# epam/Zstandard

Measured on AMD Instinct MI355X. Metric: GiB/s compress @ level 3, 64 KiB chunks, higher is better.
Workload: dtype u8; 1 GPU; 4096 independent 65536 B chunks per GPU per step, level 3, BASELINE config[1] shape (Silesia unavailable offline -> Zipf-token log stream, SURVEY 8d); chunks_per_gpu=4096, chunk_bytes=65536, level=3, parallelism=chunks sharded over 1 GPU(s), no collective in the data path

## Files before the change

### zstandard_amd/csrc/lz_kernels.hip

```cpp
#include "zsmi_device.h"
#include "zsmi_scratch.h"
#include <type_traits>

#ifndef ZS_CAND_G
#define ZS_CAND_G 8
#endif
#ifndef ZS_CAND_G_BIG
#define ZS_CAND_G_BIG 16
#endif
#define ZS_CAND_GOF(TLOG) ((TLOG) > ZS_TABLE_LOG_SMALL ? ZS_CAND_G_BIG : ZS_CAND_G)
#ifndef ZS_CAND_DEPTH
#define ZS_CAND_DEPTH 2
#endif
#define ZS_CAND_WAVES(NT) (3 * (NT))
#define ZS_CAND_ROW 65u
#define ZS_CAND_LDS(TLOG, NT) ((size_t)(NT) * (4u << (TLOG)) + 3u * (NT) * ZS_CAND_GOF(TLOG) * ZS_CAND_ROW * 4u + (NT) * 256u + 3u * 16u * 8u + 32u)
#define ZS_SLOT_EMPTY 0xFFFFFFFFu
__device__ __forceinline__ uint32_t zs_hash_short(uint32_t lo, uint32_t hi) { return __umul24(lo, 0x9E3779u) + __umul24(__builtin_amdgcn_alignbit(hi, lo, 16), 0x85EBCBu); }
__device__ __forceinline__ uint32_t zs_hash_long(uint32_t lo, uint32_t hi)
{ return __umul24(lo, 0x9E3779u) + __umul24(__builtin_amdgcn_alignbit(hi, lo, 24), 0x85EBCBu) + __umul24(hi >> 16, 0xC2B2AFu); }

template <int TLOG, int NT, bool PFX = false>
__global__ void __launch_bounds__(64 * ZS_CAND_WAVES(NT))
k_lz_candidates(const uint8_t *__restrict__ src, const ZsUnitDesc *__restrict__ units, uint32_t block0,
                uint16_t *__restrict__ distAll, uint8_t *__restrict__ distHiAll, uint32_t *__restrict__ candCount,
                const ZsCDictEntry *__restrict__ dictTab = nullptr, const uint32_t *__restrict__ unitDict = nullptr,
                const uint32_t *__restrict__ liveUnits = nullptr)
{
    static_assert(!PFX || TLOG == ZS_TABLE_LOG_BIG, "a prefixed unit spans up to 128 KiB of positions");
    if (liveUnits && blockIdx.x >= *liveUnits) return;
    const uint32_t *dictImg = nullptr; uint32_t pfx = 0;
    if constexpr (PFX) {
        const ZsCDictEntry &de = dictTab[unitDict ? unitDict[blockIdx.x] : 0u];
        dictImg = de.img; pfx = (uint32_t)__builtin_amdgcn_readfirstlane((int)de.pfx);
    }
    extern __shared__ __attribute__((aligned(16))) uint32_t candLds[];
    constexpr bool BIG = TLOG > ZS_TABLE_LOG_SMALL;
    constexpr uint32_t G = ZS_CAND_GOF(TLOG), GP = G * 64u, H = G / NT;
    constexpr uint32_t M = ZS_CAND_DEPTH;
    constexpr uint32_t LPS = 64u / G;
    constexpr uint32_t WD = G / 4u + 2u;
    static_assert(G == 8 || G == 16, "a hasher lane takes G consecutive positions of a group: 8 or 16");
    const uint32_t wave = (uint32_t)__builtin_amdgcn_readfirstlane((int)(threadIdx.x >> 6)), lane = threadIdx.x & 63u;
    const uint32_t tab = (wave < NT) ? wave : ((wave < 2 * NT) ? wave - NT : wave - 2 * NT);
    uint32_t *T = candLds + ((size_t)tab << TLOG);
    uint32_t *opnd = candLds + ((size_t)NT << TLOG);
    constexpr uint32_t ROW = ZS_CAND_ROW, GR = G * ROW;
    constexpr uint32_t RING = 3u * NT * GR;
    uint64_t *runMarks = reinterpret_cast<uint64_t *>(opnd + RING + NT * 64u);
    uint32_t *runFlag = opnd + RING + NT * 64u + 3u * 16u * 2u;
    const ZsUnitDesc ud = units[blockIdx.x];
    const uint8_t *s = src + ud.srcOff;
    const uint32_t n = ud.size;
    const size_t slot = (size_t)(ud.firstBlock - block0);
    uint16_t *dist = zs_block_dist(distAll, slot);
    uint8_t *distHi = zs_block_dist_hi(distHiAll, slot);
    const uint32_t hashable = (n >= 8) ? n - 7 : 0;
    const uint32_t nGroups = (hashable + GP - 1) / GP;
    if (threadIdx.x < 2) zs_block_cand(candCount, slot, threadIdx.x) = 0;
    if (nGroups == 0) return;
    if (n >= 16 && (n & 15u) == 0) {
        uint4 f;
        __builtin_memcpy(&f, s, 16);
        const uint32_t splat = (f.x & 0xFFu) * 0x01010101u;
        if (((f.x ^ splat) | (f.y ^ splat) | (f.z ^ splat) | (f.w ^ splat)) == 0) {
            if (threadIdx.x == 0) candLds[0] = 0;
            __syncthreads();
            uint32_t mixed = 0;
            for (uint32_t i = threadIdx.x * 16u; i < n && !mixed; i += ZS_CAND_WAVES(NT) * 64u * 16u) {
                uint4 v;
                __builtin_memcpy(&v, s + i, 16);
                mixed = (v.x ^ splat) | (v.y ^ splat) | (v.z ^ splat) | (v.w ^ splat);
            }
            if (mixed) candLds[0] = 1u;
            __syncthreads();
            const bool uniform = candLds[0] == 0;
            __syncthreads();
            if (uniform) return;
        }
    }
    const uint32_t dummyBase = ((uint32_t)(NT - tab) << TLOG) + RING + tab * 64u;
    auto mergeRead = [&](uint32_t g, uint32_t (&mS)[H], uint32_t (&mL)[H]) {
        const uint32_t *xb = opnd + (size_t)(g % 3u) * NT * GR + (NT > 1 ? tab * H : 0u) * ROW + lane;
        #pragma unroll
        for (uint32_t uu = 0; uu < H; uu++) { mS[uu] = xb[uu * ROW]; mL[uu] = (NT > 1) ? xb[GR + uu * ROW] : 0u; }
    };
    uint32_t found = 0;
    const uint32_t matchlessBelow = n >> ZS_MATCHLESS_SHIFT;
    auto mergeStore = [&](uint32_t g, const uint32_t (&mS)[H], const uint32_t (&mL)[H]) {
        const uint32_t sbase = g * GP + ((NT > 1) ? tab * H * 64u : 0u);
        uint64_t hiMine = 0;
        #pragma unroll
        for (uint32_t uu = 0; uu < H; uu++) {
            const uint32_t dm = (NT > 1) ? (mL[uu] ? mL[uu] : mS[uu]) : mS[uu];
            if (BIG) { const uint64_t hi = __ballot((dm >> 16) != 0); if (lane == uu) hiMine = hi; }
            if (found < matchlessBelow) {
                if ((g + 1u) * GP <= hashable) found += (uint32_t)__popcll(__ballot(dm != 0));
                else found += (uint32_t)__popcll(__ballot(dm != 0 && sbase + uu * 64 + lane < hashable));
            }
            dist[sbase + uu * 64 + lane] = (uint16_t)dm;
        }
        if (BIG && lane < H) *reinterpret_cast<uint64_t *>(distHi + ((sbase + lane * 64) >> 3)) = hiMine;
    };
    if (wave >= 2 * NT) {
        __syncthreads(); __syncthreads();
        for (uint32_t i = 2; i <= nGroups + 1; i++) {
            uint32_t mS[H], mL[H];
            mergeRead(i - 2, mS, mL);
            if (__builtin_amdgcn_readfirstlane((int)runFlag[((i - 2) % 3u) * 2u + tab])) {
                if (lane == 0) runFlag[((i - 2) % 3u) * 2u + tab] = 0;
                #pragma unroll
                for (uint32_t uu = 0; uu < H; uu++) {
                    const uint64_t marks = runMarks[((i - 2) % 3u) * 16u + ((NT > 1) ? tab * H : 0u) + uu];
                    if ((marks >> lane) & 1ull) { if (NT > 1) mL[uu] = 1u; else mS[uu] = 1u; }
                }
            }
            mergeStore(i - 2, mS, mL);
            __syncthreads();
        }
        if (lane == 0) zs_block_cand(candCount, slot, tab) = found;
        return;
    }

    if (wave < NT) {
        if constexpr (PFX) {
            uint4 *t4 = reinterpret_cast<uint4 *>(T);
            const uint4 *img4 = reinterpret_cast<const uint4 *>(dictImg + ((size_t)tab << TLOG));
            #pragma unroll 8
            for (uint32_t i = lane; i < (1u << TLOG) / 4; i += 64) t4[i] = img4[i];
        } else {
            uint4 *t4 = reinterpret_cast<uint4 *>(T);
            const uint4 e = make_uint4(ZS_SLOT_EMPTY, ZS_SLOT_EMPTY, ZS_SLOT_EMPTY, ZS_SLOT_EMPTY);
            #pragma unroll 8
            for (uint32_t i = lane; i < (1u << TLOG) / 4; i += 64) t4[i] = e;
        }
        uint32_t ringSlot = 0;
        __syncthreads();
        for (uint32_t i = 1; i <= nGroups; i++) {
            uint32_t *ob = opnd + ((size_t)ringSlot * NT + tab) * GR + lane;
            const uint32_t base = (i - 1) * GP + lane + (PFX ? pfx : 0u);
            uint32_t op[G], entry[G], old[G];
            #pragma unroll
            for (uint32_t u = 0; u < G; u++) op[u] = ob[u * ROW];
            #pragma unroll
            for (uint32_t u = 0; u < G; u++) {
                uint32_t pu = base + u * 64u;
                asm volatile("" : "+v"(pu));
                entry[u] = (op[u] & 0xFFFE0000u) | pu;
                old[u] = atomicExch(&T[op[u] & 0xFFFFu], entry[u]);
            }
            #pragma unroll
            for (uint32_t u = 0; u < G; u++) {
                const uint32_t x = old[u] ^ entry[u], dd = entry[u] - old[u];
                ob[u * ROW] = (max(x, dd) < (1u << 17)) ? dd : 0u;
            }
            ringSlot = (ringSlot == 2u) ? 0u : ringSlot + 1u;
            __syncthreads();
        }
        __syncthreads();
        return;
    }

    auto run = [&](auto roleTag) {
        constexpr bool LONG = decltype(roleTag)::value;
        const uint32_t stepOfLane = lane / LPS, l0 = (lane % LPS) * G;
        const uint32_t wbase = stepOfLane * ROW + l0;
        const uint32_t last8 = n - 8;
        auto loadGroup = [&](uint32_t g, uint32_t (&w)[WD]) {
            const uint32_t o = g * GP + lane * G;
            #pragma unroll
            for (uint32_t k = 0; k < WD / 2; k++) {
                const uint32_t ok = o + 8u * k, oc = min(ok, last8);
                const uint64_t v = zs_load64(s + oc) >> (8u * min(ok - oc, 7u));
                w[2 * k] = (uint32_t)v; w[2 * k + 1] = (uint32_t)(v >> 32);
            }
        };
        uint32_t bufA[M][WD], bufB[M][WD];
        auto loadM = [&](uint32_t g0, uint32_t (&buf)[M][WD]) {
            #pragma unroll
            for (uint32_t k = 0; k < M; k++) loadGroup(min(g0 + k, nGroups), buf[k]);
        };
        auto iter = [&](auto wholeTag, uint32_t i, const uint32_t (&w)[WD]) {
            constexpr bool WHOLE = decltype(wholeTag)::value;
            const uint32_t ringSlot = i % 3u;
            if (i < nGroups) {
                uint32_t *ob = opnd + ((size_t)ringSlot * NT + tab) * GR + wbase;
                const uint32_t pbase = i * GP + lane * G;
                #pragma unroll
                for (uint32_t u = 0; u < G; u++) {
                    const uint32_t k = u >> 2, sh = u & 3u;
                    const uint32_t lo = sh ? __builtin_amdgcn_alignbyte(w[k + 1], w[k], sh) : w[k];
                    const uint32_t hi = sh ? __builtin_amdgcn_alignbyte(w[min(k + 2, WD - 1)], w[k + 1], sh) : w[k + 1];
                    uint32_t h = LONG ? zs_hash_long(lo, hi) : zs_hash_short(lo, hi);
                    asm volatile("" : "+v"(h));
                    const uint32_t r = __builtin_amdgcn_alignbit(h, h, 32 - TLOG);
                    ob[u] = (WHOLE || pbase + u < hashable) ? (r & (0xFFFE0000u | ((1u << TLOG) - 1u))) : ((r & 0xFFFE0000u) | (dummyBase + l0 + u));
                }
                bool flat = false;
                uint64_t flatLanes = 0;
                if (WHOLE && __ballot(w[0] == w[1])) {
                    uint32_t diff = w[0] ^ __builtin_amdgcn_alignbyte(w[0], w[0], 1);
                    #pragma unroll
                    for (uint32_t k = 1; k < WD; k++) diff |= w[k] ^ w[k - 1];
                    flat = diff == 0;
                    flatLanes = __ballot(flat);
                }
                if (flatLanes) {
                    const uint32_t key = flat ? ((w[0] & 0xFFu) | 0x100u) : 0u;
                    const uint32_t keyBelow = (uint32_t)__builtin_amdgcn_update_dpp(0, (int)key, 0x138, 0xF, 0xF, true);
                    const uint32_t keyAbove = (uint32_t)__builtin_amdgcn_update_dpp(0, (int)key, 0x130, 0xF, 0xF, true);
                    const bool markFirst = flat && keyBelow == key && (lane % LPS) != 0u;
                    const bool innerLast = flat && keyAbove == key && (lane % LPS) != LPS - 1u;
                    if (flat) {
                        uint32_t h = LONG ? zs_hash_long(w[0], w[1]) : zs_hash_short(w[0], w[1]);
                        asm volatile("" : "+v"(h));
                        const uint32_t away = (__builtin_amdgcn_alignbit(h, h, 32 - TLOG) & 0xFFFE0000u) | (dummyBase + l0);
                        if (markFirst) ob[0] = away;
                        #pragma unroll
                        for (uint32_t u = 1; u + 1 < G; u++) ob[u] = away + u;
                        if (innerLast) ob[G - 1] = away + (G - 1);
                    }
                    if (!LONG) {
                        if (lane < NT) runFlag[ringSlot * 2u + lane] = 1u;
                        const uint32_t bits = flat ? (((1u << G) - 2u) | (markFirst ? 1u : 0u)) : 0u;
                        if (G == 8) reinterpret_cast<uint8_t *>(runMarks + ringSlot * 16u)[lane] = (uint8_t)bits;
                        else reinterpret_cast<uint16_t *>(runMarks + ringSlot * 16u)[lane] = (uint16_t)bits;
                    }
                }
            }
            __syncthreads();
        };
        auto step = [&](uint32_t i, const uint32_t (&w)[WD]) {
            if (i > nGroups + 1) return;
            if ((i + 1) * GP + 8u <= n) iter(std::true_type{}, i, w); else iter(std::false_type{}, i, w);
        };
        if (!LONG && lane < 6u) runFlag[lane] = 0;
        loadM(0, bufA);
        for (uint32_t g0 = 0; g0 <= nGroups + 1; g0 += 2 * M) {
            loadM(g0 + M, bufB);
            #pragma unroll
            for (uint32_t k = 0; k < M; k++) step(g0 + k, bufA[k]);
            loadM(g0 + 2 * M, bufA);
            #pragma unroll
            for (uint32_t k = 0; k < M; k++) step(g0 + M + k, bufB[k]);
        }
    };
    if (tab == 0) run(std::false_type{}); else run(std::true_type{});
}

__global__ void __launch_bounds__(1024)
k_lz_dict_tables(const ZsCDictEntry entry, ZsCDictEntry *__restrict__ entryOut)
{
    constexpr int TLOG = ZS_TABLE_LOG_BIG;
    __shared__ uint32_t T[1u << TLOG];
    const uint32_t tab = blockIdx.x, tid = threadIdx.x;
    const uint8_t *__restrict__ pre = entry.pre; const uint32_t pfx = entry.pfx; uint32_t *__restrict__ img = const_cast<uint32_t *>(entry.img);
    if (tab == 0 && tid == 0) *entryOut = entry;
    for (uint32_t i = tid; i < (1u << TLOG); i += 1024) T[i] = 0;
    __syncthreads();
    const uint32_t hashable = pfx >= 8 ? pfx - 7 : 0;
    for (uint32_t p = tid; p < hashable; p += 1024) {
        const uint64_t v = zs_load64(pre + p);
        const uint32_t lo = (uint32_t)v, hi = (uint32_t)(v >> 32);
        const uint32_t h = tab ? zs_hash_long(lo, hi) : zs_hash_short(lo, hi);
        const uint32_t r = __builtin_amdgcn_alignbit(h, h, 32 - TLOG);
        atomicMax(&T[r & ((1u << TLOG) - 1u)], ((p + 1u) << 15) | (r >> 17));
    }
    __syncthreads();
    uint32_t *out = img + ((size_t)tab << TLOG);
    for (uint32_t i = tid; i < (1u << TLOG); i += 1024) {
        const uint32_t k = T[i];
        out[i] = k ? (((k & 0x7FFFu) << 17) | ((k >> 15) - 1u)) : ZS_SLOT_EMPTY;
    }
}

#ifndef ZS_WALK_MINW
#define ZS_WALK_MINW 1
#endif
#define ZS_WALK_WGRP(WLOG) ((WLOG) >= 9 ? 4 : 2)
#ifndef ZS_WALK_LPW_256
#define ZS_WALK_LPW_256 2
#endif
#ifndef ZS_WALK_LPW_512
#define ZS_WALK_LPW_512 4
#endif
#define ZS_WALK_LPW(WLOG) ((WLOG) >= 9 ? ZS_WALK_LPW_512 : ZS_WALK_LPW_256)
#define ZS_WALK_THREADS(BIG, WLOG) ((((BIG) ? ZS_UNIT_MAX : ZS_BLOCK_MAX) >> (WLOG)) * ZS_WALK_LPW(WLOG))
static_assert(ZS_WALK_THREADS(false, 8) / ZS_WALK_LPW(8) == (ZS_BLOCK_MAX >> 8) && ZS_WALK_THREADS(false, 9) / ZS_WALK_LPW(9) == (ZS_BLOCK_MAX >> 9) &&
              ZS_WALK_THREADS(true, 8) / ZS_WALK_LPW(8) == (ZS_UNIT_MAX >> 8) && ZS_WALK_THREADS(true, 9) / ZS_WALK_LPW(9) == (ZS_UNIT_MAX >> 9),
              "a walker per walk range of a unit of full capacity");
#define ZS_WALK_KERNEL(LOOK, REPW, BIG, WLOG) k_lz_walk<ZS_WALK_LPW(WLOG), ZS_WALK_WGRP(WLOG), LOOK, REPW, BIG, ZS_WALK_THREADS(BIG, WLOG)>
#ifndef ZS_WALK_SKEW
#define ZS_WALK_SKEW  24u
#endif
#define ZS_WALK_FRONT 48u
#define ZS_WALK_TAIL  144u
#define ZS_WALK_SRCBYTES(CAPB) ((((CAPB) + ZS_WALK_TAIL + ZS_WALK_SKEW * (((CAPB) + ZS_WALK_TAIL) / 256u + 1u)) + 15u) & ~15u)
#define ZS_WALK_LDS(CAPB) ((CAPB) / 8 + 16 + ZS_WALK_FRONT + ZS_WALK_SRCBYTES(CAPB) + 16 + 1024)

typedef const __attribute__((address_space(3))) uint32_t *ZsLdsU32;
template <int K>
__device__ __forceinline__ void lds_span(uint32_t byteOff, uint32_t (&out)[K])
{
    ZsLdsU32 d = (ZsLdsU32)(uintptr_t)(byteOff & ~3u);
    uint32_t w[K + 1];
    #pragma unroll
    for (int k = 0; k <= K; k++) w[k] = d[k];
    const uint32_t sh = byteOff & 3u;
    #pragma unroll
    for (int k = 0; k < K; k++) out[k] = __builtin_amdgcn_alignbyte(w[k + 1], w[k], sh);
}
template <int I, int K>
__device__ __forceinline__ uint32_t span_at(const uint32_t (&v)[K])
{
    if constexpr ((I & 3) == 0) return v[I >> 2];
    else return __builtin_amdgcn_alignbyte(v[(I >> 2) + 1], v[I >> 2], I & 3);
}
__device__ __forceinline__ uint32_t zs_agree16(const uint32_t (&a)[4], const uint32_t (&b)[4])
{
    const uint64_t x0 = (uint64_t)(a[0] ^ b[0]) | ((uint64_t)(a[1] ^ b[1]) << 32), x1 = (uint64_t)(a[2] ^ b[2]) | ((uint64_t)(a[3] ^ b[3]) << 32);
    const uint32_t n0 = x0 ? ((uint32_t)__builtin_ctzll(x0) >> 3) : 8u;
    const uint32_t n1 = x1 ? ((uint32_t)__builtin_ctzll(x1) >> 3) : 8u;
    return (n0 < 8u) ? n0 : 8u + n1;
}
template <int LPW> __device__ __forceinline__ uint32_t walker_or(uint32_t v)
{
    if constexpr (LPW >= 2) v |= (uint32_t)__builtin_amdgcn_update_dpp(0, (int)v, 0xB1, 0xF, 0xF, false);
    if constexpr (LPW == 4) v |= (uint32_t)__builtin_amdgcn_update_dpp(0, (int)v, 0x4E, 0xF, 0xF, false);
    return v;
}
template <int LPW> __device__ __forceinline__ int walker_max(int v)
{
    if constexpr (LPW >= 2) v = max(v, __builtin_amdgcn_update_dpp(0, v, 0xB1, 0xF, 0xF, false));
    if constexpr (LPW == 4) v = max(v, __builtin_amdgcn_update_dpp(0, v, 0x4E, 0xF, 0xF, false));
    return v;
}
template <int LPW> __device__ __forceinline__ uint32_t walker_min(uint32_t v)
{
    if constexpr (LPW >= 2) v = min(v, (uint32_t)__builtin_amdgcn_update_dpp(0, (int)v, 0xB1, 0xF, 0xF, false));
    if constexpr (LPW == 4) v = min(v, (uint32_t)__builtin_amdgcn_update_dpp(0, (int)v, 0x4E, 0xF, 0xF, false));
    return v;
}
template <int NT, int DIR>
__device__ __forceinline__ uint32_t block_scan_max(uint32_t v, uint32_t *wv, uint32_t tid, uint32_t *total)
{
    const uint32_t lane = tid & 63u, wave = tid >> 6;
    #pragma unroll
    for (int d = 1; d < 64; d <<= 1) {
        const uint32_t o = (uint32_t)(DIR > 0 ? __shfl_up((int)v, d) : __shfl_down((int)v, d));
        if (DIR > 0 ? (int)lane >= d : (int)lane + d < 64) v = max(v, o);
    }
    __syncthreads();
    if (lane == (DIR > 0 ? 63u : 0u)) wv[wave] = v;
    __syncthreads();
    uint32_t pre = 0, all = 0;
    #pragma unroll
    for (uint32_t k = 0; k < NT / 64; k++) { const uint32_t x = wv[k]; all = max(all, x); if (DIR > 0 ? k < wave : k > wave) pre = max(pre, x); }
    *total = all;
    return max(v, pre);
}
__device__ __forceinline__ uint32_t zs_nonzero8(const uint4 d)
{
    typedef uint16_t u16x2 __attribute__((ext_vector_type(2)));
    const u16x2 one = { 1, 1 };
    (void)one;
    auto nz = [&](uint32_t w) { uint32_t r; asm("v_pk_min_u16 %0, %1, %2" : "=v"(r) : "v"(w), "v"(0x00010001u)); return r; };
    const uint32_t v = nz(d.x) | (nz(d.y) << 2) | (nz(d.z) << 4) | (nz(d.w) << 6);
    return (v | (v >> 15)) & 0xFFu;
}

#ifdef ZS_WALK_PROFILE
#define WPROF_STAMP(k) { __builtin_amdgcn_sched_barrier(0); unsigned long long t_; asm volatile("s_waitcnt vmcnt(0) lgkmcnt(0)\n\ts_memtime %0\n\ts_waitcnt lgkmcnt(0)" : "=s"(t_) :: "memory"); __builtin_amdgcn_sched_barrier(0); wprof[k] += t_ - wlast; wlast = t_; }
#else
#define WPROF_STAMP(k)
#endif
#define ZS_WALK_KERNEL_PFX(LOOK, REPW, WLOG) k_lz_walk<ZS_WALK_LPW(WLOG), ZS_WALK_WGRP(WLOG), LOOK, REPW, true, ZS_WALK_THREADS(false, WLOG), true>
template <int LPW, int WGRP, int LOOK, int REPWIN, bool BIG, int NT, bool PFX = false>
__global__ void __launch_bounds__(NT, BIG ? 1 : ZS_WALK_MINW)
k_lz_walk(const uint8_t *__restrict__ src, const ZsUnitDesc *__restrict__ units, uint32_t block0,
          const uint16_t *__restrict__ distAll, const uint8_t *__restrict__ distHiAll,
          uint2 *__restrict__ recAll, uint32_t junkSlot, uint4 *__restrict__ resAll, int rangeLogArg, const uint32_t *__restrict__ candCount,
          const ZsCDictEntry *__restrict__ dictTab = nullptr, const uint32_t *__restrict__ unitDict = nullptr,
          const uint32_t *__restrict__ liveUnits = nullptr)
{
    static_assert(!PFX || BIG, "a prefixed unit is staged in the 128 KiB layout");
    if (liveUnits && blockIdx.x >= *liveUnits) return;
    const uint8_t *pre = nullptr; uint32_t pfx = 0;
    if constexpr (PFX) {
        const ZsCDictEntry &de = dictTab[unitDict ? unitDict[blockIdx.x] : 0u];
        pre = de.pre; pfx = (uint32_t)__builtin_amdgcn_readfirstlane((int)de.pfx);
    }
    constexpr uint32_t CAP = BIG ? ZS_UNIT_MAX : ZS_BLOCK_MAX;
    constexpr uint32_t CPL = LOOK / LPW, RPL = REPWIN / LPW, GPL = WGRP / LPW;
    static_assert((LPW == 1 || LPW == 2 || LPW == 4) && WGRP % LPW == 0 && LOOK % LPW == 0 && REPWIN % LPW == 0 && CPL >= 1 && RPL >= 1 && LOOK <= 8 && REPWIN <= 8, "a walker's lanes share the groups and candidates evenly");
    static_assert(NT >= 64 && NT % 64 == 0 && NT * GPL * 16 <= CAP / 8, "the exchange buffer holds 16 bytes a lane and group");
    extern __shared__ __attribute__((aligned(16))) uint8_t walkLds[];
    constexpr uint32_t SRC = CAP / 8 + 16 + ZS_WALK_FRONT;
    auto lposv = [](uint32_t v) { return SRC + v + (uint32_t)__mul24((int)v >> 8, (int)ZS_WALK_SKEW); };
    const uint32_t vb = PFX ? pfx : 0u;
    auto lpos = [&](uint32_t p) { return lposv(p + vb); };
    auto stage16 = [&](uint32_t i, const uint4 v) {
        uint8_t *d = walkLds + lposv(i);
        *reinterpret_cast<uint2 *>(d) = make_uint2(v.x, v.y); *reinterpret_cast<uint2 *>(d + 8) = make_uint2(v.z, v.w);
        const uint32_t o = i & 255u;
        if (o == 0) { *reinterpret_cast<uint2 *>(d - ZS_WALK_SKEW) = make_uint2(v.x, v.y); *reinterpret_cast<uint2 *>(d - ZS_WALK_SKEW + 8) = make_uint2(v.z, v.w); }
        else if (o == 16) *reinterpret_cast<uint2 *>(d - ZS_WALK_SKEW) = make_uint2(v.x, v.y);
    };
    const uint32_t tid = threadIdx.x, lane = tid & 63u;
    const uint32_t rangeLog = (uint32_t)rangeLogArg, R = 1u << rangeLog;
    const ZsUnitDesc ud = units[blockIdx.x];
    const uint32_t slot = ud.firstBlock - block0;
    const uint8_t *s = src + ud.srcOff;
    const uint32_t n = ud.size;
    const uint16_t *dist = zs_block_dist(distAll, slot);
    const uint8_t *distHi = zs_block_dist_hi(distHiAll, slot);
    uint4 *xbuf = reinterpret_cast<uint4 *>(walkLds);
    const uint32_t xw = (tid & ~63u) * GPL;
    const uint32_t safeAddr = (xw + lane) * 16u;
    uint32_t *mixedWord = reinterpret_cast<uint32_t *>(walkLds + SRC + ZS_WALK_SRCBYTES(CAP)) + 1;
    uint4 *res = zs_block_range_results(resAll, slot);
    uint8_t *xhi = reinterpret_cast<uint8_t *>(mixedWord + 3);
    uint2 *recs = zs_block_walk_records(recAll, slot);
    const uint32_t sub = lane & (LPW - 1u);
#ifdef ZS_WALK_PROFILE
    unsigned long long wprof[10] = { 0, 0, 0, 0, 0, 0, 0, 0, 0, 0 }, wlast;
    asm volatile("s_memtime %0\n\ts_waitcnt lgkmcnt(0)" : "=s"(wlast) :: "memory");
#endif

    if (zs_block_cand(candCount, slot, 0) + zs_block_cand(candCount, slot, 1) < (n >> ZS_MATCHLESS_SHIFT)) {
        const uint32_t nRanges = (n + R - 1) >> rangeLog, perBlockLog = 16u - rangeLog;
        for (uint32_t r = tid; r < nRanges; r += NT) res[zs_unit_range_result(r, perBlockLog)] = make_uint4(0, 0, 0, 0);
        return;
    }
    uint32_t mixed = 0;
    if (tid < (ZS_WALK_FRONT - ZS_WALK_SKEW) / 4) reinterpret_cast<uint32_t *>(walkLds + SRC - ZS_WALK_FRONT)[tid] = 0;
    if (tid == 0) *mixedWord = 0;
    __syncthreads();
    if constexpr (PFX) {
        const uint32_t end = pfx + n, splat = (n ? (uint32_t)s[0] : 0u) * 0x01010101u;
        for (uint32_t i = tid * 16; i < end + ZS_WALK_TAIL && i + 16 <= CAP + ZS_WALK_TAIL; i += NT * 16) {
            uint4 w = make_uint4(0, 0, 0, 0);
            if (i + 16 <= pfx) __builtin_memcpy(&w, pre + i, 16);
            else if (i >= pfx && i + 16 <= end) {
                __builtin_memcpy(&w, s + (i - pfx), 16);
                mixed |= (w.x ^ splat) | (w.y ^ splat) | (w.z ^ splat) | (w.w ^ splat);
            } else if (i < end) {
                uint8_t b[16];
                for (uint32_t k = 0; k < 16; k++) {
                    const uint32_t v = i + k;
                    b[k] = v < pfx ? pre[v] : (v < end ? s[v - pfx] : (uint8_t)0);
                    if (v >= pfx && v < end && b[k] != (uint8_t)splat) mixed = 1;
                }
                __builtin_memcpy(&w, b, 16);
            }
            stage16(i, w);
        }
        if ((n & 15u) != 0 || n < 16) mixed = 1;
    } else {
        constexpr uint32_t PER = (CAP / 16 + NT - 1) / NT;
        const uint32_t nFull = n & ~15u;
        uint4 v[PER];
        const uint32_t splat = (n ? (uint32_t)s[0] : 0u) * 0x01010101u;
        #pragma unroll
        for (uint32_t k = 0; k < PER; k++) {
            const uint32_t i = (tid + k * NT) * 16;
            const uint32_t ii = (i + 16 <= nFull) ? i : 0u;
            v[k] = make_uint4(0, 0, 0, 0);
            if (nFull >= 16) __builtin_memcpy(&v[k], s + ii, 16);
        }
        #pragma unroll
        for (uint32_t k = 0; k < PER; k++) {
            const uint32_t i = (tid + k * NT) * 16;
            if (i + 16 <= nFull) stage16(i, v[k]);
            mixed |= (v[k].x ^ splat) | (v[k].y ^ splat) | (v[k].z ^ splat) | (v[k].w ^ splat);
        }
        if (n != nFull || n < 16) mixed = 1;
        for (uint32_t i = nFull + tid * 16; i < n + ZS_WALK_TAIL; i += NT * 16) {
            uint4 w = make_uint4(0, 0, 0, 0);
            if (i < n) {
                uint64_t lo = 0, hi = 0;
                for (uint32_t k = 0; k < 16 && i + k < n; k++) { const uint64_t c = s[i + k]; if (k < 8) lo |= c << (8 * k); else hi |= c << (8 * (k - 8)); }
                w = make_uint4((uint32_t)lo, (uint32_t)(lo >> 32), (uint32_t)hi, (uint32_t)(hi >> 32));
            }
            if (i + 16 <= CAP + ZS_WALK_TAIL) stage16(i, w);
        }
    }
#if defined(ZS_WALK_STOP) && ZS_WALK_STOP == 1
    if (n) return;
#endif
    const uint32_t hashable = (n >= 8) ? n - 7 : 0;
    if (mixed) *mixedWord = 1u;
    __syncthreads();
    if (*mixedWord == 0) {
        const uint32_t nRanges = (n + R - 1) >> rangeLog, perBlockLog = 16u - rangeLog;
        for (uint32_t r = tid; r < nRanges; r += NT) res[zs_unit_range_result(r, perBlockLog)] = make_uint4(0, 0, 0, 0);
        return;
    }
    WPROF_STAMP(0)

    {
        const uint32_t nRanges = (n + R - 1) >> rangeLog;
        bool active = false;
        uint32_t ip = 0, anchor = 0, scanEnd = 0, limit = 0, rep0 = 0, rep1 = 0, nseq = 0, lastOff = 0, blockBase = 0;
        uint2 heldRec = make_uint2(0, 0);
        const uint32_t perBlockLog = 16u - rangeLog;
        typedef __attribute__((address_space(3))) uint4 *ZsLdsU4;
        const uint32_t xwaveLds = (uint32_t)__builtin_amdgcn_readfirstlane((int)(uint32_t)(uintptr_t)(ZsLdsU4)(xbuf + xw));
        asm volatile("s_mov_b32 m0, %0\n\ts_nop 0" :: "s"(xwaveLds) : "memory");
        uint32_t gh[GPL] = {};
        auto loadGroup = [&](uint32_t p) {
            #pragma unroll
            for (uint32_t k = 0; k < GPL; k++) {
                const uint32_t g = (p >> 3) + sub + LPW * k;
                const uint16_t *gsrc = dist + (size_t)g * 8u;
                if constexpr (GPL == 1) asm volatile("global_load_lds_dwordx4 %0, off" :: "v"(gsrc) : "memory");
                else asm volatile("s_mov_b32 m0, %1\n\ts_nop 0\n\tglobal_load_lds_dwordx4 %0, off" :: "v"(gsrc), "s"(xwaveLds + k * 1024u) : "memory");
                if (BIG) gh[k] = (uint32_t)distHi[g];
            }
        };
        const uint32_t r = tid / LPW;
        const uint32_t recBase = r << (rangeLog - 2u), resAt = zs_unit_range_result(r, perBlockLog);
        if (r < nRanges) {
            const uint32_t start = r << rangeLog;
            const uint32_t blockStart = start & ~(ZS_BLOCK_MAX - 1);
            const uint32_t blockEnd = blockStart + min(n - blockStart, ZS_BLOCK_MAX);
            const uint32_t end = min(start + R, blockEnd);
            limit = min(end + ZS_CROSS_MAX, blockEnd);
            scanEnd = (blockEnd - blockStart >= 16) ? min(end, hashable) : 0;
            ip = start; anchor = start; blockBase = blockStart;
            active = ip < scanEnd;
            if (!active && sub == 0) res[resAt] = make_uint4(0, 0, 0, 0);
            if (active) loadGroup(ip);
        }
        asm volatile("s_waitcnt vmcnt(0)" ::: "memory");
        while (__any(active)) {
            WPROF_STAMP(1)
#ifdef ZS_WALK_PROFILE
            wprof[8] += 1; wprof[9] += (unsigned long long)__popcll(__ballot(active));
#endif
            const uint32_t wend = min((ip & ~7u) + 8u * WGRP, scanEnd);
            uint32_t rm0 = 0, rm1 = 0;
            {
                const bool t0 = active && rep0 != 0 && ip + vb >= rep0, t1 = active && rep1 != 0 && ip + vb >= rep1;
                const uint32_t p0 = ip + sub * RPL;
                constexpr int SP = (RPL + 3 + 3) / 4;
                uint32_t a[SP] = {}, b[SP] = {}, c[SP] = {};
                {
                    const bool tr = t0 || t1;
                    lds_span<SP>(tr ? lpos(p0) : safeAddr, a);
                    lds_span<SP>(tr ? lpos(t0 ? p0 - rep0 : p0) : safeAddr, b);
                    lds_span<SP>(tr ? lpos(t1 ? p0 - rep1 : p0) : safeAddr, c);
                }
                auto tryAt = [&](auto iTag) {
                    constexpr int I = decltype(iTag)::value;
                    const uint32_t q = p0 + I;
                    const bool ok = q < wend && q + 4 <= limit;
                    const uint32_t av = span_at<I>(a);
                    if (t0 && ok && av == span_at<I>(b)) rm0 |= 1u << (sub * RPL + I);
                    if (t1 && ok && av == span_at<I>(c)) rm1 |= 1u << (sub * RPL + I);
                };
                tryAt(std::integral_constant<int, 0>{});
                if constexpr (RPL >= 2) tryAt(std::integral_constant<int, 1>{});
                if constexpr (RPL >= 4) { tryAt(std::integral_constant<int, 2>{}); tryAt(std::integral_constant<int, 3>{}); }
                if constexpr (RPL >= 8) { tryAt(std::integral_constant<int, 4>{}); tryAt(std::integral_constant<int, 5>{}); tryAt(std::integral_constant<int, 6>{}); tryAt(std::integral_constant<int, 7>{}); }
                rm0 = walker_or<LPW>(rm0); rm1 = walker_or<LPW>(rm1);
                rm1 &= ~rm0;
            }
            WPROF_STAMP(2)
            asm volatile("s_waitcnt vmcnt(0)" ::: "memory");
            uint32_t m = 0;
            #pragma unroll
            for (uint32_t k = 0; k < GPL; k++) {
                const uint4 gd = xbuf[xw + 64u * k + lane];
                if (BIG) xhi[xw + 64u * k + lane] = (uint8_t)gh[k];
                m |= (zs_nonzero8(gd) | gh[k]) << (8u * (sub + LPW * k));
            }
            m = walker_or<LPW>(m) >> (ip & 7u);
            if (active) m = (m & (0xFFFFFFFFu >> (32u - (wend - ip)))) | rm0 | rm1; else m = 0;
            {
                const uint32_t skip = sub * CPL;
                if constexpr ((LPW - 1) * CPL >= 4) { uint32_t t = m & (m - 1); t &= t - 1; t &= t - 1; t &= t - 1; m = (skip & 4u) ? t : m; }
                if constexpr ((((LPW - 1) * CPL) & 2) != 0 || (LPW == 4 && CPL == 2)) { uint32_t t = m & (m - 1); t &= t - 1; m = (skip & 2u) ? t : m; }
                if constexpr ((CPL & 1) != 0) { const uint32_t t = m & (m - 1); m = (skip & 1u) ? t : m; }
            }
            uint32_t idx[CPL], off[CPL], dv[CPL]; bool have[CPL], isRep[CPL];
            #pragma unroll
            for (uint32_t c = 0; c < CPL; c++) {
                have[c] = m != 0;
                idx[c] = have[c] ? (uint32_t)__builtin_ctz(m) : 0u;
                m &= m - 1;
                const uint32_t q = ip + idx[c];
                const uint32_t j = (q >> 3) - (ip >> 3);
                const uint32_t owner = xw + 64u * (j / LPW) + (lane & ~(LPW - 1u)) + (j % LPW);
                dv[c] = reinterpret_cast<const uint16_t *>(xbuf + owner)[q & 7u];
                if (BIG) dv[c] |= (((uint32_t)xhi[owner] >> (q & 7u)) & 1u) << 16;
            }
            #pragma unroll
            for (uint32_t c = 0; c < CPL; c++) asm volatile("" : "+v"(dv[c]));
            #pragma unroll
            for (uint32_t c = 0; c < CPL; c++) {
                const bool r0 = ((rm0 >> idx[c]) & 1u) != 0, r1 = ((rm1 >> idx[c]) & 1u) != 0;
                isRep[c] = have[c] && (r0 || r1);
                off[c] = r0 ? rep0 : (r1 ? rep1 : dv[c]);
                if (!have[c]) off[c] = 0;
            }
            WPROF_STAMP(3)
            int bestKey = 0; uint32_t bestPack = 0, bestOff = 0;
            uint32_t sa[CPL][3], sb[CPL][3];
            #pragma unroll
            for (uint32_t c = 0; c < CPL; c++) {
                const uint32_t q = ip + idx[c];
                #pragma unroll
                for (int k = 0; k < 3; k++) { sa[c][k] = 0; sb[c][k] = 0; }
                const bool tr = have[c];
                lds_span<3>(tr ? lpos(q - 4) : safeAddr, sa[c]);
                lds_span<3>(tr ? lpos(q - off[c] - 4) : safeAddr, sb[c]);
            }
            #pragma unroll
            for (uint32_t c = 0; c < CPL; c++) asm volatile("" : "+v"(sa[c][0]), "+v"(sa[c][1]), "+v"(sa[c][2]), "+v"(sb[c][0]), "+v"(sb[c][1]), "+v"(sb[c][2]));
            #pragma unroll
            for (uint32_t c = 0; c < CPL; c++) {
                const uint32_t q = ip + idx[c];
                const uint32_t (&a)[3] = sa[c], (&b)[3] = sb[c];
                const uint32_t xb = a[0] ^ b[0], x0 = a[1] ^ b[1], x1 = a[2] ^ b[2];
                const uint32_t f0 = x0 ? (uint32_t)__builtin_ctz(x0) : 32u, f1 = x1 ? (uint32_t)__builtin_ctz(x1) : 32u;
                const uint32_t fwd = min(((x0 ? f0 : 32u + f1)) >> 3, limit - q);
                const uint32_t maxBack = min(min(q - anchor, q + vb - off[c]), ZS_BCAP);
                const uint32_t back = min(xb ? ((uint32_t)__builtin_clz(xb) >> 3) : 4u, maxBack);
                if (have[c] && fwd >= (isRep[c] ? ZS_REPMIN : ZS_MINMATCH)) {
                    const int gain = (int)(4u * fwd + 8u * back) - (isRep[c] ? 0 : (int)zs_highbit(off[c] + 1)) - 5 * (int)idx[c];
                    const int key = ((gain + 2048) << 3) | (int)(7u - (sub * CPL + c));
                    if (key > bestKey) { bestKey = key; bestPack = idx[c] | (fwd << 8) | (back << 16); bestOff = off[c]; }
                }
            }
            const int best = walker_max<LPW>(bestKey);
            const bool took = active && best != 0;
            const uint32_t packed = walker_or<LPW>(bestKey == best ? bestPack : 0u), boff = walker_or<LPW>(bestKey == best ? bestOff : 0u);
            const uint32_t bq = ip + (packed & 0xFFu), bback = packed >> 16;
            uint32_t bfwd = (packed >> 8) & 0xFFu;
            WPROF_STAMP(4)
            const bool extend = took && bfwd == ZS_FCAP && (limit - bq) > ZS_FCAP;
            bool need = extend;
            uint32_t pos = bq + ZS_FCAP;
            while (__any(need)) {
                uint32_t e = 0xFFFFFFFFu;
                if (need) {
                    const uint32_t cap = limit - pos, fo = 16u * sub;
                    uint32_t nb = 0;
                    if (fo < cap) {
                        uint32_t a[4], b[4];
                        lds_span<4>(lpos(pos + fo), a);
                        lds_span<4>(lpos(pos - boff + fo), b);
                        nb = zs_agree16(a, b);
                    }
                    if (nb < 16u || fo + 16u >= cap) e = min(fo + nb, cap);
                }
                e = walker_min<LPW>(e);
                if (need) {
                    if (e != 0xFFFFFFFFu) { pos += e; need = false; }
                    else pos += 16u * LPW;
                }
            }
            if (extend) bfwd = pos - bq;
            WPROF_STAMP(5)
            const uint32_t recStart = bq - bback, recLl = recStart - anchor;
            const uint2 rec = make_uint2((recStart - blockBase) | ((bback + bfwd) << 17), boff | (recLl << 17));
            const bool rot = took && boff != rep0;
            rep1 = rot ? rep0 : rep1; rep0 = rot ? boff : rep0;
            nseq += took ? 1u : 0u;
            lastOff = took ? boff : lastOff;
            ip = took ? bq + bfwd : (active ? wend : ip);
            anchor = took ? ip : anchor;
            const bool odd = (nseq & 1u) != 0, done = active && ip >= scanEnd, first = sub == 0;
            if (took && !odd && first) *reinterpret_cast<uint4 *>(recs + recBase + nseq - 2) = make_uint4(heldRec.x, heldRec.y, rec.x, rec.y);
            heldRec.x = (took && odd) ? rec.x : heldRec.x; heldRec.y = (took && odd) ? rec.y : heldRec.y;
            if (done && odd && first) recs[recBase + nseq - 1] = heldRec;
            if (done && first) res[resAt] = make_uint4(nseq, nseq ? anchor - blockBase : 0u, lastOff, 0u);
            active = active && !done;
            if (active) loadGroup(ip);
            WPROF_STAMP(6)
        }
    }
    WPROF_STAMP(1)
#ifdef ZS_WALK_PROFILE
    __syncthreads();
    if (lane == 0) { unsigned long long *o = zs_res_lend_walk_profile(resAll, junkSlot) + ((size_t)blockIdx.x * (NT / 64) + (tid >> 6)) * 10; for (int k = 0; k < 10; k++) o[k] = wprof[k]; }
#endif
}

__global__ void __launch_bounds__(256)
k_lz_stitch(const ZsBlockDesc *__restrict__ blocks, const uint2 *__restrict__ recAll, const uint4 *__restrict__ resAll,
            ZsSeqRec *__restrict__ seqAll, uint32_t *__restrict__ hdrAll, int rangeLogArg, const uint32_t *__restrict__ liveBlocks = nullptr)
{
    constexpr int NT = 256;
    if (liveBlocks && blockIdx.x >= *liveBlocks) return;
    __shared__ __attribute__((aligned(16))) uint32_t sa[4 * 256 + 16];
    uint32_t *sKept = sa, *sStart = sa + 256, *sWave = sa + 1024, *sTot = sa + 1028, *sMl = sa + 1032, *sEnd = sa + 1036;
    uint2 *sInfo = reinterpret_cast<uint2 *>(sa + 512);
    const uint32_t tid = threadIdx.x, lane = tid & 63u;
    const uint32_t rangeLog = (uint32_t)rangeLogArg;
    const uint32_t slot = blockIdx.x;
    const uint32_t NRB = ZS_BLOCK_MAX >> rangeLog;
    const uint2 *recs = zs_block_walk_records(recAll, slot);
    const uint4 *res = zs_block_range_results(resAll, slot);
    {
        const uint32_t bStart = 0, bi = 0;
        const uint32_t bN = blocks[slot].size;
        const uint32_t bEnd = bN;
        const uint32_t t = tid;
        const bool mine = t < NRB;
        const bool walked = mine && bN >= 16 && (t << rangeLog) < bN;
        const uint4 rr = walked ? res[t] : make_uint4(0, 0, 0, 0);
        const uint32_t ns = rr.x, le = rr.y;
        const uint32_t rs = min(bStart + (t << rangeLog), bEnd);
        const uint2 *rp = recs + ((bStart + (t << rangeLog)) >> 2);
        uint32_t total;
        const uint32_t key = ns ? ((le << 9) | (511u - t)) : 0u;
        const uint32_t incl = block_scan_max<NT, 1>(key, sWave, tid, &total);
        uint32_t excl = (uint32_t)__shfl_up((int)incl, 1);
        if (lane == 0) { excl = 0; for (uint32_t k = 0; k < (tid >> 6); k++) excl = max(excl, sWave[k]); }
        const uint32_t own = max(excl >> 9, bStart), reachAll = max(total >> 9, bStart);
        const uint32_t definer = 511u - (excl & 511u);
#if defined(ZS_STITCH_STOP) && ZS_STITCH_STOP == 2
        if (bN) return;
#endif
        uint32_t f = 0, fStart = 0, fEnd = 0, fOff = 0;
        if (ns && own >= rs) {
            if (le <= own) f = ns;
            else {
                const uint4 r01 = *reinterpret_cast<const uint4 *>(rp);
                auto endOf = [](uint32_t x) { return (x & 0x1FFFFu) + (x >> 17); };
                uint2 rec = make_uint2(r01.x, r01.y), nxt = make_uint2(r01.z, r01.w);
                bool haveNxt = ns > 1;
                if (endOf(r01.x) > own) f = 0;
                else if (ns > 1 && endOf(r01.z) > own) { f = 1; rec = nxt; haveNxt = false; }
                else {
                    uint32_t lo = 2, hi = ns - 1;
                    while (lo < hi) { const uint32_t mid = (lo + hi) >> 1; if (endOf(rp[mid].x) > own) hi = mid; else lo = mid + 1; }
                    f = lo; rec = rp[f]; haveNxt = false;
                }
                uint32_t st = rec.x & 0x1FFFFu, en = endOf(rec.x);
                if (st < own && en - own < ZS_MINMATCH) {
                    f++;
                    if (f < ns) { rec = haveNxt ? nxt : rp[f]; st = rec.x & 0x1FFFFu; en = endOf(rec.x); }
                }
                fStart = max(st, own); fEnd = en; fOff = rec.y & 0x1FFFFu;
            }
        }
        const bool keptAny = f < ns;
        sKept[t] = (keptAny ? 1u : 0u) | (rr.z << 1);
        __syncthreads();
        const uint32_t defWord = sKept[excl != 0 ? definer : 0u];
        const bool joined = keptAny && excl != 0 && own >= rs && fStart == own && fOff == (defWord >> 1) && (defWord & 1u) != 0;
        const uint32_t fOut = f + (joined ? 1u : 0u), cnt = ns - fOut;
        const bool stopper = ns && le > own && !(joined && cnt == 0);
        uint32_t total2;
        const uint32_t key2 = stopper ? (((512u - t) << 18) | (joined ? fEnd : own)) : 0u;
        const uint32_t sfx = block_scan_max<NT, -1>(key2, sWave, tid, &total2);
        uint32_t sfxEx = (uint32_t)__shfl_down((int)sfx, 1);
        if (lane == 63) { sfxEx = 0; for (uint32_t k = (tid >> 6) + 1; k < NT / 64; k++) sfxEx = max(sfxEx, sWave[k]); }
        const uint32_t chainEnd = sfxEx ? (sfxEx & 0x3FFFFu) : reachAll;
        const uint32_t wave = tid >> 6;
        const uint32_t cntIncl = wave_incl_scan(cnt);
        if (lane == 63) sTot[wave] = cntIncl;
        sInfo[t] = make_uint2(own | (fOut << 17), chainEnd | (ns << 17));
        __syncthreads();
        uint32_t start = cntIncl - cnt, nseq = 0;
        #pragma unroll
        for (uint32_t k = 0; k < NT / 64; k++) { const uint32_t x = sTot[k]; nseq += x; if (k < wave) start += x; }
        sStart[t] = start;
        __syncthreads();
#if defined(ZS_STITCH_STOP) && ZS_STITCH_STOP == 1
        if (bN) return;
#endif
        constexpr uint32_t PB = 4;
        ZsSeqRec *out = zs_block_seqs(seqAll, slot);
        uint2 recN[PB]; uint32_t ownN[PB], endN[PB];
        auto request = [&](uint32_t base) {
            #pragma unroll
            for (uint32_t q = 0; q < PB; q++) {
                const uint32_t d = base + NT * q + tid;
                recN[q] = make_uint2(0, 0); ownN[q] = 0; endN[q] = 0;
                if (d < nseq) {
                    uint32_t jr = 0;
                    #pragma unroll
                    for (uint32_t stepb = NT / 2; stepb >= 1; stepb >>= 1) if (d >= sStart[jr + stepb]) jr += stepb;
                    const uint2 info = sInfo[jr];
                    const uint32_t at = d - sStart[jr], k = (info.x >> 17) + at;
                    ownN[q] = (info.x & 0x1FFFFu) | (at == 0 ? 0x80000000u : 0u);
                    endN[q] = (info.y & 0x1FFFFu) | (k + 1 == (info.y >> 17) ? 0x80000000u : 0u);
                    recN[q] = recs[(jr << (rangeLog - 2)) + k];
                }
            }
        };
        request(0);
        #pragma unroll
        for (uint32_t q = 0; q < PB; q++) asm volatile("" : "+v"(recN[q].x), "+v"(recN[q].y));
        uint32_t mlSum = 0;
        for (uint32_t base = 0; base < nseq; base += NT * PB) {
            uint2 recC[PB]; uint32_t ownC[PB], endC[PB];
            #pragma unroll
            for (uint32_t q = 0; q < PB; q++) { recC[q] = recN[q]; ownC[q] = ownN[q]; endC[q] = endN[q]; }
            if (base + NT * PB < nseq) request(base + NT * PB);
            #pragma unroll
            for (uint32_t q = 0; q < PB; q++) {
                const uint32_t d = base + NT * q + tid;
                if (d < nseq) {
                    const uint2 rec = recC[q];
                    uint32_t st = rec.x & 0x1FFFFu, ml = rec.x >> 17;
                    const uint32_t off = rec.y & 0x1FFFFu, en = st + ml;
                    if (ownC[q] >> 31) {
                        const uint32_t ownj = ownC[q] & 0x1FFFFu;
                        if (st < ownj) { st = ownj; ml = en - st; }
                    }
                    if (endC[q] >> 31) ml = (endC[q] & 0x1FFFFu) - st;
                    ZsSeqRec w; w.x = zs_rec_x(ml, off); w.y = zs_rec_y(off, st);
                    out[d] = w;
                    mlSum += ml;
                    if (d + 1 == nseq) sEnd[0] = st + ml;
                }
            }
        }
        const uint32_t mlWave = wave_sum(mlSum);
        if (lane == 0) sMl[wave] = mlWave;
        __syncthreads();
        if (tid == 0) {
            uint32_t covered = 0;
            for (uint32_t k = 0; k < NT / 64; k++) covered += sMl[k];
            ZsBlockHdr h; h.nseq = nseq; h.trailing = bN - (nseq ? sEnd[0] : 0u); h.lits = bN - covered; h.pad = 0;
            zs_block_hdr(hdrAll, slot) = h;
        }
    }
}
```

Before: 148.0 GiB/s.

## Split hasher positions across waves and compute short and long hashes together

Before, each hasher wave computed a single hash kind (short or long) over G positions per lane. Now each hasher wave covers only G/NT positions per lane and produces both the short and long hash operands for them, sharing the common first multiply and the loaded window. This cuts per-lane window loads and duplicated byte-alignment work. In exchange, run-mark and flag writes become per-wave sub-slices, which adds a DPP merge path for 4-position lanes and more subtle indexing.

```diff
diff --git a/zstandard_amd/csrc/lz_kernels.hip b/zstandard_amd/csrc/lz_kernels.hip
--- a/zstandard_amd/csrc/lz_kernels.hip
+++ b/zstandard_amd/csrc/lz_kernels.hip
@@ -16,9 +16,12 @@
 #define ZS_CAND_ROW 65u
 #define ZS_CAND_LDS(TLOG, NT) ((size_t)(NT) * (4u << (TLOG)) + 3u * (NT) * ZS_CAND_GOF(TLOG) * ZS_CAND_ROW * 4u + (NT) * 256u + 3u * 16u * 8u + 32u)
 #define ZS_SLOT_EMPTY 0xFFFFFFFFu
-__device__ __forceinline__ uint32_t zs_hash_short(uint32_t lo, uint32_t hi) { return __umul24(lo, 0x9E3779u) + __umul24(__builtin_amdgcn_alignbit(hi, lo, 16), 0x85EBCBu); }
-__device__ __forceinline__ uint32_t zs_hash_long(uint32_t lo, uint32_t hi)
-{ return __umul24(lo, 0x9E3779u) + __umul24(__builtin_amdgcn_alignbit(hi, lo, 24), 0x85EBCBu) + __umul24(hi >> 16, 0xC2B2AFu); }
+__device__ __forceinline__ uint32_t zs_hash_first(uint32_t lo) { return __umul24(lo, 0x9E3779u); }
+__device__ __forceinline__ uint32_t zs_hash_short_from(uint32_t first, uint32_t lo, uint32_t hi) { return first + __umul24(__builtin_amdgcn_alignbit(hi, lo, 16), 0x85EBCBu); }
+__device__ __forceinline__ uint32_t zs_hash_long_from(uint32_t first, uint32_t lo, uint32_t hi)
+{ return first + __umul24(__builtin_amdgcn_alignbit(hi, lo, 24), 0x85EBCBu) + __umul24(hi >> 16, 0xC2B2AFu); }
+__device__ __forceinline__ uint32_t zs_hash_short(uint32_t lo, uint32_t hi) { return zs_hash_short_from(zs_hash_first(lo), lo, hi); }
+__device__ __forceinline__ uint32_t zs_hash_long(uint32_t lo, uint32_t hi) { return zs_hash_long_from(zs_hash_first(lo), lo, hi); }
 
 template <int TLOG, int NT, bool PFX = false>
 __global__ void __launch_bounds__(64 * ZS_CAND_WAVES(NT))
@@ -38,9 +41,10 @@
     constexpr bool BIG = TLOG > ZS_TABLE_LOG_SMALL;
     constexpr uint32_t G = ZS_CAND_GOF(TLOG), GP = G * 64u, H = G / NT;
     constexpr uint32_t M = ZS_CAND_DEPTH;
-    constexpr uint32_t LPS = 64u / G;
-    constexpr uint32_t WD = G / 4u + 2u;
-    static_assert(G == 8 || G == 16, "a hasher lane takes G consecutive positions of a group: 8 or 16");
+    constexpr uint32_t PL = H;
+    constexpr uint32_t LPS = 64u / PL;
+    constexpr uint32_t NB = PL + 7u, WD = (NB + 3u) / 4u;
+    static_assert(PL == 4 || PL == 8 || PL == 16, "a hasher lane takes 4, 8 or 16 consecutive positions of a group");
     const uint32_t wave = (uint32_t)__builtin_amdgcn_readfirstlane((int)(threadIdx.x >> 6)), lane = threadIdx.x & 63u;
     const uint32_t tab = (wave < NT) ? wave : ((wave < 2 * NT) ? wave - NT : wave - 2 * NT);
     uint32_t *T = candLds + ((size_t)tab << TLOG);
@@ -79,7 +83,7 @@
             if (uniform) return;
         }
     }
-    const uint32_t dummyBase = ((uint32_t)(NT - tab) << TLOG) + RING + tab * 64u;
+    auto dummyBase = [&](uint32_t t) { return ((uint32_t)(NT - t) << TLOG) + RING + t * 64u; };
     auto mergeRead = [&](uint32_t g, uint32_t (&mS)[H], uint32_t (&mL)[H]) {
         const uint32_t *xb = opnd + (size_t)(g % 3u) * NT * GR + (NT > 1 ? tab * H : 0u) * ROW + lane;
         #pragma unroll
@@ -161,18 +165,24 @@
         return;
     }
 
-    auto run = [&](auto roleTag) {
-        constexpr bool LONG = decltype(roleTag)::value;
-        const uint32_t stepOfLane = lane / LPS, l0 = (lane % LPS) * G;
-        const uint32_t wbase = stepOfLane * ROW + l0;
-        const uint32_t last8 = n - 8;
+    {
+        constexpr bool LONG = NT > 1;
+        const uint32_t lbase = tab * H * 64u + lane * PL;
+        const uint32_t l0 = (lane % LPS) * PL;
+        const uint32_t wbase = (lbase / 64u) * ROW + l0;
+        const uint32_t dummyS = dummyBase(0) + l0, dummyL = dummyBase(NT - 1) + l0;
+        const uint32_t last8 = n - 8, last4 = n - 4;
         auto loadGroup = [&](uint32_t g, uint32_t (&w)[WD]) {
-            const uint32_t o = g * GP + lane * G;
+            const uint32_t o = g * GP + lbase;
             #pragma unroll
             for (uint32_t k = 0; k < WD / 2; k++) {
                 const uint32_t ok = o + 8u * k, oc = min(ok, last8);
                 const uint64_t v = zs_load64(s + oc) >> (8u * min(ok - oc, 7u));
                 w[2 * k] = (uint32_t)v; w[2 * k + 1] = (uint32_t)(v >> 32);
+            }
+            if (WD & 1u) {
+                const uint32_t ok = o + 4u * (WD - 1u), oc = min(ok, last4);
+                w[WD - 1] = zs_load32(s + oc) >> (8u * min(ok - oc, 3u));
             }
         };
         uint32_t bufA[M][WD], bufB[M][WD];
@@ -184,24 +194,32 @@
             constexpr bool WHOLE = decltype(wholeTag)::value;
             const uint32_t ringSlot = i % 3u;
             if (i < nGroups) {
-                uint32_t *ob = opnd + ((size_t)ringSlot * NT + tab) * GR + wbase;
-                const uint32_t pbase = i * GP + lane * G;
+                uint32_t word = ringSlot * NT * GR + wbase;
+                asm volatile("" : "+v"(word));
+                uint32_t *obS = opnd + word, *obL = obS + (NT - 1) * GR;
+                const uint32_t pbase = i * GP + lbase;
+                auto operand = [&](uint32_t h, bool inserted, uint32_t dummy) {
+                    asm volatile("" : "+v"(h));
+                    const uint32_t r = __builtin_amdgcn_alignbit(h, h, 32 - TLOG);
+                    return inserted ? (r & (0xFFFE0000u | ((1u << TLOG) - 1u))) : ((r & 0xFFFE0000u) | dummy);
+                };
                 #pragma unroll
-                for (uint32_t u = 0; u < G; u++) {
+                for (uint32_t u = 0; u < PL; u++) {
                     const uint32_t k = u >> 2, sh = u & 3u;
                     const uint32_t lo = sh ? __builtin_amdgcn_alignbyte(w[k + 1], w[k], sh) : w[k];
                     const uint32_t hi = sh ? __builtin_amdgcn_alignbyte(w[min(k + 2, WD - 1)], w[k + 1], sh) : w[k + 1];
-                    uint32_t h = LONG ? zs_hash_long(lo, hi) : zs_hash_short(lo, hi);
-                    asm volatile("" : "+v"(h));
-                    const uint32_t r = __builtin_amdgcn_alignbit(h, h, 32 - TLOG);
-                    ob[u] = (WHOLE || pbase + u < hashable) ? (r & (0xFFFE0000u | ((1u << TLOG) - 1u))) : ((r & 0xFFFE0000u) | (dummyBase + l0 + u));
+                    const uint32_t first = zs_hash_first(lo);
+                    const bool inserted = WHOLE || pbase + u < hashable;
+                    obS[u] = operand(zs_hash_short_from(first, lo, hi), inserted, dummyS + u);
+                    if (LONG) obL[u] = operand(zs_hash_long_from(first, lo, hi), inserted, dummyL + u);
                 }
                 bool flat = false;
                 uint64_t flatLanes = 0;
                 if (WHOLE && __ballot(w[0] == w[1])) {
                     uint32_t diff = w[0] ^ __builtin_amdgcn_alignbyte(w[0], w[0], 1);
                     #pragma unroll
-                    for (uint32_t k = 1; k < WD; k++) diff |= w[k] ^ w[k - 1];
+                    for (uint32_t k = 1; k + 1 < WD; k++) diff |= w[k] ^ w[k - 1];
+                    diff |= (w[WD - 1] ^ w[WD - 2]) & (0xFFFFFFFFu >> (8u * (4u * WD - NB)));
                     flat = diff == 0;
                     flatLanes = __ballot(flat);
                 }
@@ -212,19 +230,27 @@
                     const bool markFirst = flat && keyBelow == key && (lane % LPS) != 0u;
                     const bool innerLast = flat && keyAbove == key && (lane % LPS) != LPS - 1u;
                     if (flat) {
-                        uint32_t h = LONG ? zs_hash_long(w[0], w[1]) : zs_hash_short(w[0], w[1]);
-                        asm volatile("" : "+v"(h));
-                        const uint32_t away = (__builtin_amdgcn_alignbit(h, h, 32 - TLOG) & 0xFFFE0000u) | (dummyBase + l0);
-                        if (markFirst) ob[0] = away;
-                        #pragma unroll
-                        for (uint32_t u = 1; u + 1 < G; u++) ob[u] = away + u;
-                        if (innerLast) ob[G - 1] = away + (G - 1);
+                        const uint32_t first = zs_hash_first(w[0]);
+                        auto sendAway = [&](uint32_t *ob, uint32_t h, uint32_t dummy) {
+                            const uint32_t away = operand(h, false, dummy);
+                            if (markFirst) ob[0] = away;
+                            #pragma unroll
+                            for (uint32_t u = 1; u + 1 < PL; u++) ob[u] = away + u;
+                            if (innerLast) ob[PL - 1] = away + (PL - 1);
+                        };
+                        sendAway(obS, zs_hash_short_from(first, w[0], w[1]), dummyS);
+                        if (LONG) sendAway(obL, zs_hash_long_from(first, w[0], w[1]), dummyL);
                     }
-                    if (!LONG) {
-                        if (lane < NT) runFlag[ringSlot * 2u + lane] = 1u;
-                        const uint32_t bits = flat ? (((1u << G) - 2u) | (markFirst ? 1u : 0u)) : 0u;
-                        if (G == 8) reinterpret_cast<uint8_t *>(runMarks + ringSlot * 16u)[lane] = (uint8_t)bits;
-                        else reinterpret_cast<uint16_t *>(runMarks + ringSlot * 16u)[lane] = (uint16_t)bits;
+                    {
+                        if (lane == 0) runFlag[ringSlot * 2u + tab] = 1u;
+                        uint32_t bits = flat ? (((1u << PL) - 2u) | (markFirst ? 1u : 0u)) : 0u;
+                        uint8_t *marks = reinterpret_cast<uint8_t *>(runMarks + ringSlot * 16u) + lbase / 8u;
+                        if (PL == 16) *reinterpret_cast<uint16_t *>(marks) = (uint16_t)bits;
+                        else if (PL == 8) *marks = (uint8_t)bits;
+                        else {
+                            bits |= (uint32_t)__builtin_amdgcn_update_dpp(0, (int)bits, 0x130, 0xF, 0xF, true) << 4;
+                            if ((lane & 1u) == 0u) *marks = (uint8_t)bits;
+                        }
                     }
                 }
             }
@@ -234,7 +260,7 @@
             if (i > nGroups + 1) return;
             if ((i + 1) * GP + 8u <= n) iter(std::true_type{}, i, w); else iter(std::false_type{}, i, w);
         };
-        if (!LONG && lane < 6u) runFlag[lane] = 0;
+        if (lane < 3u) runFlag[lane * 2u + tab] = 0;
         loadM(0, bufA);
         for (uint32_t g0 = 0; g0 <= nGroups + 1; g0 += 2 * M) {
             loadM(g0 + M, bufB);
@@ -244,8 +270,7 @@
             #pragma unroll
             for (uint32_t k = 0; k < M; k++) step(g0 + M + k, bufB[k]);
         }
-    };
-    if (tab == 0) run(std::false_type{}); else run(std::true_type{});
+    }
 }
 
 __global__ void __launch_bounds__(1024)
```

Measured after the change: 147.8 GiB/s. No clear change (-0.1%).
